# ndjinga/CirculantPreconditioner

Hardware: AMD Instinct MI355X
Metric: PCApply/s on 256^3 complex grid (higher is better)
Workload: dtype c128 (f64 complex); 1 GPU; 256x256x256 c128 circulant PCApply, transport symbol lambda=(0.6, 0.15, 0.02); global_batch=1, parallelism=single GPU

## Files before the change

circulantpreconditioner_amd/csrc/cfp_three_pass.hip:

```cpp
#include "cfp_fft_device.h"
#include "cfp_lane.h"
#include "cfp_three_pass.h"

#include <hip/hip_ext.h>

#ifndef CFP_REAL_MID_XCD
#define CFP_REAL_MID_XCD 1
#endif

#define TP_LAUNCH(K, G, B, S, ...)                                                                    \
  do {                                                                                                \
    if (g_stamp.start || g_stamp.stop)                                                                \
      hipExtLaunchKernelGGL(K, G, B, 0, S, g_stamp.start, g_stamp.stop, 0, __VA_ARGS__);              \
    else                                                                                              \
      hipLaunchKernelGGL(K, G, B, 0, S, __VA_ARGS__);                                                 \
  } while (0)

namespace cfp {

namespace {

__device__ __forceinline__ cd dft4_dif(cd v, int q) {
  const cd p = dpp_c<DPP_XOR2>(v);
  cd t = (q & 2) ? csub(p, v) : cadd(v, p);
  if (q == 3) t = mul_mi(t);
  const cd r = dpp_c<DPP_XOR1>(t);
  return (q & 1) ? csub(r, t) : cadd(t, r);
}
__device__ __forceinline__ cd dft4_dit(cd v, int q) {
  const cd r = dpp_c<DPP_XOR1>(v);
  cd u = (q & 1) ? csub(r, v) : cadd(v, r);
  if (q == 3) u = mul_mi(u);
  const cd p = dpp_c<DPP_XOR2>(u);
  return (q & 2) ? csub(p, u) : cadd(u, p);
}
template <int N2>
__device__ __forceinline__ int brev(int j) {
  if constexpr (N2 == 16) return ((j & 1) << 3) | ((j & 2) << 1) | ((j & 4) >> 1) | (j >> 3);
  return N2 == 4 ? ((j & 1) << 1) | (j >> 1) : ((j & 1) << 2) | (j & 2) | (j >> 2);
}
__device__ __forceinline__ int xcd_unit(int it, int G) {
  const int b = it % G;
  return it - b + (b & 7) * (G >> 3) + (b >> 3);
}

__device__ __forceinline__ int idx(int i) {
  asm volatile("" : "+v"(i));
  return i;
}

template <int FLAGS>
__device__ __forceinline__ unsigned char gload_u8(const unsigned char* p) {
  if constexpr ((FLAGS & F_NT_LD) != 0) return __builtin_nontemporal_load(p);
  return *p;
}

constexpr int r0_of(int n, int pts) { return n > pts ? r0_of(n / pts, pts) : n; }

}

#ifndef CFP_POST_NT
#define CFP_POST_NT 1
#endif
constexpr int kPostLoadFlags = CFP_POST_NT ? F_NT_LD : 0;

enum { PR_NO_Y2 = 1, PR_NO_ZMATH = 2, PR_NO_XCHG = 4, PR_NO_LOAD = 8, PR_NO_STORE = 16,
       PR_PRIO = 32 ,
       PR_ZMAJOR = 64  };

template <bool INV, int FLAGS, int N1, int TN, int PTS = 16, bool XS = true, bool LP = false, int BLK = 0,
          bool XCD = false, int PROBE = 0, int FUSE = 0>
__global__ void __launch_bounds__(N1 * (TN / PTS)) __attribute__((amdgpu_waves_per_eu(4)))
k_tp_rows(const cd* in, cd* out, TPArgs a, int nunits) {
#ifndef CFP_KEXP
  static_assert(PROBE == 0, "timing probes are built in tools/kexp only");
#endif
  constexpr int N2 = TN / N1, TR = TN / PTS, NT = N1 * TR, TY = N1 / PTS;
  constexpr bool PRE = !INV && FUSE == 1, POST = INV && FUSE > 0;
  constexpr int NP = POST ? FUSE : 1;
  static_assert(!POST || NP <= TP_POST_MAX, "post dots: at most TP_POST_MAX vectors");
  static_assert(FUSE == 0 || (BLK == 0 && PROBE == 0), "fused work: natural layout, product kernels");
  constexpr bool BL = BLK > 0;
  constexpr int BX = BL ? BLK : 1, BW = N2 * BX;
  static_assert(!LP || (TY == 2 && TN % 32 == 0), "lane pairs: two threads per column, 32 columns per wave");
  static_assert(!BL || (TR % BX == 0 && ((N2 == 8 && (BX == 4 || BX == 8)) || (N2 == 16 && (BX == 2 || BX == 8)))),
                "blocked layout: 4 or 8 x times 8 y2, or 2 or 8 x times 16 y2");
  constexpr int RS = TN + TN / 16;
  constexpr int F = FLAGS | (XS ? F_SPLIT_LDS : 0) | F_LDS_SYNC;
  constexpr int FA = F & ~F_WAVE_LDS;
  static_assert(!(FLAGS & F_WAVE_LDS) || 64 % TR == 0, "wave-local rows: whole rows per wave");
  __shared__ __attribute__((aligned(16))) double lds[N1 * RS * (XS ? 1 : 2)];
  __shared__ cd tw_l[N1];
  __shared__ cd pre_tab_l[PRE ? 3 * TP_PRE_MAX_CLS : 1];
  __shared__ unsigned pre_mk_l[PRE ? TP_PRE_MAX_CLS + 1 : 1];
  __shared__ const unsigned char* pre_cls_l[1];
  __shared__ cd pre_edge_l[PRE ? NT : 1];
  __shared__ double post_l[POST ? 2 * NP * (NT / 64) : 1];
  __shared__ const cd* post_ptr_l[POST ? NP : 1];
  __shared__ int post_n_l[2];
  const int tid = threadIdx.x;
  if constexpr (POST) {
    for (int i = tid; i < 2 * NP * (NT / 64); i += NT) post_l[i] = 0.0;
    if (tid < NP) post_ptr_l[tid] = a.post_v[tid];
    if (tid == 0) {
      post_n_l[0] = a.post_nv;
      post_n_l[1] = a.post_self;
    }
  }
  for (int i = tid; i < N1; i += NT) tw_l[i] = a.tw[N2 * i];
  if constexpr (PRE) {
    for (int c = tid; c < a.pre_ncls; c += NT) {
      const unsigned mk = a.pre_mask[c];
      unsigned dense = 0;
      pre_tab_l[3 * c] = pre_tab_l[3 * c + 1] = pre_tab_l[3 * c + 2] = make_cd(0.0, 0.0);
      for (int k = 0; k < a.pre_nd; ++k)
        if ((mk >> k) & 1u) {
          const int slot = a.pre_off[k] + 1;
          pre_tab_l[3 * c + slot] = a.pre_tab[c * a.pre_nd + k];
          dense |= 1u << slot;
        }
      pre_mk_l[c] = dense;
    }
    if (tid == 0) {
      unsigned all = 0;
      for (int k = 0; k < a.pre_nd; ++k) all |= 1u << (a.pre_off[k] + 1);
      pre_mk_l[TP_PRE_MAX_CLS] = all | (a.pre_cls_x ? 8u : 0u);
      pre_cls_l[0] = a.pre_cls_x ? a.pre_cls_x : a.pre_cls;
    }
  }
  if constexpr (LP || PRE || POST) __syncthreads();
  const int x0 = LP ? (tid & 31) + 32 * (tid >> 6) : tid % TN, ty0 = LP ? (tid >> 5) & 1 : tid / TN;
  const int r0 = tid / TR, tx0 = tid % TR;
  const int lnyl = a.lnyl ? a.lnyl : ilog2(TN);
  const int nyl = 1 << lnyl;
  const auto crow = [&](int z, int y) -> i64 {
    return (i64)(y >> lnyl) * a.chunk + ((i64)z << lnyl) * TN + (i64)(y & (nyl - 1)) * TN;
  };
  const auto load = [&](int u, cd* v) {
    const int x = idx(x0), ty = idx(ty0);
    if constexpr ((PROBE & PR_NO_LOAD) != 0) {
#pragma unroll
      for (int m = 0; m < PTS; ++m) v[m] = make_cd(x + m, ty + u);
      return;
    }
    if (INV) {
      const cd* const src = BL ? in + crow(u / N2, N2 * ty) + (u % N2) * BX + (x / BX) * BW + x % BX
                               : in + crow(u / N2, u % N2 + N2 * ty) + x;
#pragma unroll
      for (int m = 0; m < PTS; ++m) v[m] = gload<FLAGS>(src + crow(0, N2 * TY * m));
    } else if constexpr (PRE) {
      static_assert(LP, "the fused stencil relies on the lane-pair layout");
      const i64 p0 = (i64)(u / N2) * TN * TN + (i64)TN * (u % N2 + N2 * ty);
      const i64 i0 = p0 + x;
      const int l32 = (int)(threadIdx.x & 31), wv = (int)(threadIdx.x >> 6);
      const unsigned slots = ((volatile unsigned*)pre_mk_l)[TP_PRE_MAX_CLS];
      const bool hm = (slots & 1u) != 0, hp = (slots & 4u) != 0;
      const unsigned char* const cls = ((const unsigned char* const volatile*)pre_cls_l)[0];
      const bool by_x = (slots & 8u) != 0;
      int cl[PTS];
      const int clx = by_x ? (int)gload_u8<FLAGS>(cls + x) : 0;
#pragma unroll
      for (int m = 0; m < PTS; ++m) {
        const i64 i = i0 + (i64)TN * N2 * TY * m;
        v[m] = gload<FLAGS>(in + i);
        cl[m] = by_x ? clx : (int)gload_u8<FLAGS>(cls + i);
      }
      cd edge = make_cd(0.0, 0.0);
      {
        const bool left = l32 < 16;
        int xe = left ? x - l32 - 1 : x - l32 + 32;
        xe = xe < 0 ? 0 : (xe > TN - 1 ? TN - 1 : xe);
        if ((left && hm) || (!left && hp)) edge = gload<FLAGS>(in + p0 + (i64)TN * N2 * TY * (l32 & 15) + xe);
      }
      __builtin_amdgcn_sched_barrier(0);
      cd* const el = pre_edge_l + 64 * wv;
      el[threadIdx.x & 63] = edge;
      __builtin_amdgcn_s_waitcnt(0xc07f);
      __builtin_amdgcn_wave_barrier();
      const auto coefs = [&](int c, cd* t) {
        t[0] = pre_tab_l[3 * c];
        t[1] = pre_tab_l[3 * c + 1];
        t[2] = pre_tab_l[3 * c + 2];
      };
      cd tx[3];
      if (by_x) coefs(clx, tx);
#pragma unroll
      for (int m = 0; m < PTS; ++m) {
        cd t[3];
        if (by_x) {
          t[0] = tx[0], t[1] = tx[1], t[2] = tx[2];
        } else {
          coefs(cl[m], t);
        }
        double ax = 0.0, ay = 0.0;
        const auto acc = [&](cd q, cd b) {
          ax = fma(q.x, b.x, fma(-q.y, b.y, ax));
          ay = fma(q.x, b.y, fma(q.y, b.x, ay));
        };
        if (hm) {
          cd bm = dpp_c<DPP_WAVE_SHR1>(v[m]);
          if (l32 == 0) bm = el[32 * ty + m];
          acc(t[0], bm);
        }
        acc(t[1], v[m]);
        if (hp) {
          cd bp = dpp_c<DPP_WAVE_SHL1>(v[m]);
          if (l32 == 31) bp = el[32 * ty + 16 + m];
          acc(t[2], bp);
        }
        v[m] = make_cd(ax, ay);
      }
    } else {
      const cd* const src = in + (i64)(u / N2) * TN * TN + x + (i64)TN * (u % N2 + N2 * ty);
#pragma unroll
      for (int m = 0; m < PTS; ++m) v[m] = gload<FLAGS>(src + (i64)TN * N2 * TY * m);
    }
    __builtin_amdgcn_sched_barrier(0);
  };
  for (int it = blockIdx.x; it < nunits; it += gridDim.x) {
    int u = XCD ? xcd_unit(it, gridDim.x) : it;
    if constexpr ((PROBE & PR_ZMAJOR) != 0) u = (u % (nunits / N2)) * N2 + u / (nunits / N2);
    cd v[PTS];
    load(u, v);
    if (INV) {
#pragma unroll
      for (int m = 0; m < PTS; ++m) v[m] = cconj(v[m]);
    }
    const auto k1_of = [](int m, int ty) {
      return LP ? (m & (PTS / 2 - 1)) + (PTS / 2) * ty + PTS * (m / (PTS / 2)) : ty + TY * m;
    };
    if constexpr ((PROBE & PR_NO_ZMATH) != 0) {
    } else if constexpr (LP) {
      dft_reg<PTS>(v);
      {
        const int ty = idx(ty0);
#pragma unroll
        for (int k = 1; k < PTS; ++k) v[k] = cmul(v[k], tw_l[k * ty]);
      }
#pragma unroll
      for (int k = 0; k < PTS / 2; ++k) swap_c<5>(v[k], v[k + PTS / 2]);
#pragma unroll
      for (int k = 0; k < PTS / 2; ++k) {
        const cd p = v[k], q = v[k + PTS / 2];
        v[k] = cadd(p, q);
        v[k + PTS / 2] = csub(p, q);
      }
    } else {
      const int x = idx(x0), ty = idx(ty0);
      fft_stages<N1, PTS, r0_of(N1, PTS), false, TN, FA>(v, lds, tw_l, x, ty, true);
      lds_barrier();
    }
    if constexpr (!(PROBE & PR_NO_XCHG)) {
      const int x = idx(x0), ty = idx(ty0), r = idx(r0), tx = idx(tx0);
      if constexpr (XS) {
#pragma unroll
        for (int half = 0; half < 2; ++half) {
#pragma unroll
          for (int m = 0; m < PTS; ++m) lds[k1_of(m, ty) * RS + x + (x >> 4)] = half ? v[m].y : v[m].x;
          lds_barrier();
#pragma unroll
          for (int m = 0; m < PTS; ++m) {
            const int xx = tx + TR * m;
            const double val = lds[r * RS + xx + (xx >> 4)];
            if (half) v[m].y = val; else v[m].x = val;
          }
          lds_barrier();
        }
      } else {
        cd* const lc = reinterpret_cast<cd*>(lds);
#pragma unroll
        for (int m = 0; m < PTS; ++m) lc[k1_of(m, ty) * RS + x + (x >> 4)] = v[m];
        lds_barrier();
#pragma unroll
        for (int m = 0; m < PTS; ++m) {
          const int xx = tx + TR * m;
          v[m] = lc[r * RS + xx + (xx >> 4)];
        }
        lds_barrier();
      }
    }
    {
      const int r = idx(r0), tx = idx(tx0);
      if constexpr (!(PROBE & PR_NO_ZMATH))
        fft_stages<TN, PTS, r0_of(TN, PTS), true, N1, F | F_TW_GLOBAL>(v, lds, a.tw, r, tx, true);
    }
    {
      const int r = idx(r0), tx = idx(tx0);
      const double sc = a.scale, sy = INV ? -sc : sc;
      if constexpr ((PROBE & PR_NO_STORE) != 0) {
        double acc = 0.0;
#pragma unroll
        for (int m = 0; m < PTS; ++m) acc += v[m].x * sc + v[m].y * sy;
        if (acc == 1.2345e300) out[tx] = make_cd(acc, 0.0);
      } else if (BL && !INV) {
        cd* dst = out + crow(u / N2, N2 * r) + (u % N2) * BX + (tx / BX) * BW + tx % BX;
#pragma unroll
        for (int m = 0; m < PTS; ++m) gstore<FLAGS>(dst + TR * N2 * m, make_cd(v[m].x * sc, v[m].y * sy));
      } else {
        const i64 e0 = (INV ? (i64)(u / N2) * TN * TN + (i64)TN * (u % N2 + N2 * r) : crow(u / N2, u % N2 + N2 * r)) + tx;
        cd* dst = out + e0;
#pragma unroll
        for (int m = 0; m < PTS; ++m) {
          v[m] = make_cd(v[m].x * sc, v[m].y * sy);
          gstore<FLAGS>(dst + TR * m, v[m]);
        }
        if constexpr (POST) {
          const int lane = tid & 63, wv = tid >> 6;
          const int pnv = ((volatile int*)post_n_l)[0], pself = ((volatile int*)post_n_l)[1];
          constexpr int QB = 4;
#pragma unroll
          for (int j = 0; j < NP; ++j) {
            if (j < pnv) {
              double sr = 0.0, si = 0.0;
              if ((pself >> j) & 1) {
#pragma unroll
                for (int m = 0; m < PTS; ++m) sr += v[m].x * v[m].x + v[m].y * v[m].y;
              } else {
                const cd* pv = ((const cd* volatile*)post_ptr_l)[j] + e0;
#pragma unroll
                for (int m0 = 0; m0 < PTS; m0 += QB) {
                  cd q[QB];
#pragma unroll
                  for (int m = 0; m < QB; ++m) q[m] = gload<kPostLoadFlags>(pv + TR * (m0 + m));
#pragma unroll
                  for (int m = 0; m < QB; ++m) {
                    const cd w = v[m0 + m];
                    sr += q[m].x * w.x + q[m].y * w.y;
                    si += q[m].x * w.y - q[m].y * w.x;
                  }
                }
              }
              sr = wave_sum_d(sr);
              si = wave_sum_d(si);
              if (lane == 0) {
                post_l[(2 * j) * (NT / 64) + wv] += sr;
                post_l[(2 * j + 1) * (NT / 64) + wv] += si;
              }
            }
          }
        }
      }
    }
    lds_barrier();
  }
  if constexpr (POST) {
    __syncthreads();
    if (tid < 2 * NP) {
      double s = 0.0;
#pragma unroll
      for (int q = 0; q < NT / 64; ++q) s += post_l[tid * (NT / 64) + q];
      a.post_partial[(size_t)blockIdx.x * 16 + tid] = s;
    }
  }
}


template <int FLAGS, int T, int N2, int TN, int PTS = 16, bool XS = true, int NX = TN, bool XCD = false,
          int BLK = 0, int PROBE = 0>
__global__ void __launch_bounds__(T * (TN / PTS)) __attribute__((amdgpu_waves_per_eu(4)))
k_tp_mid(cd* data, TPArgs a, int nunits) {
#ifndef CFP_KEXP
  static_assert(PROBE == 0, "timing probes are built in tools/kexp only");
#endif
  constexpr int N1 = TN / N2, TZ = TN / PTS, NT = T * TZ, XT = T / N2, NXT = NX / XT;
  constexpr int F = FLAGS | (XS ? F_SPLIT_LDS : 0) | F_LDS_SYNC;
  static_assert(N2 == 4 || N2 == 8 || N2 == 16, "the y2 DFT runs across 4, 8 or 16 lanes");
  static_assert(BLK == 0 || (BLK % XT == 0 && NX % BLK == 0), "blocks of whole x tiles");
  __shared__ __attribute__((aligned(16))) double lds[T * TN * (XS ? 1 : 2)];
  __shared__ cd tw_l[TN];
  const int tid = threadIdx.x;
  for (int i = tid; i < TN; i += NT) tw_l[i] = a.tw[i];
  const int c0 = tid & (T - 1), tz0 = tid / T;
  const i64 zs = (i64)NX << (a.lnyl ? a.lnyl : ilog2(TN));
  struct Col {
    cd* col;
    int y2, xk;
    cd w, w8, w16;
  };
  const auto column = [&](int u) {
    int c = c0, tz = tz0;
    asm volatile("" : "+v"(c), "+v"(tz));
    Col q;
    const int xt = u % NXT, k1 = u / NXT;
    q.y2 = c & (N2 - 1);
    q.xk = xt * XT + c / N2;
    q.col = BLK ? data + (i64)NX * N2 * k1 + (q.xk / BLK) * (N2 * BLK) + q.y2 * BLK + q.xk % BLK + zs * tz
                : data + q.xk + (i64)NX * (q.y2 + N2 * k1) + zs * tz;
    q.w = a.tw[(q.y2 * (a.k1_off + k1)) & (TN - 1)];
    q.w8 = a.tw[(TN / 8) * (q.y2 & 3)];
    if constexpr (N2 == 16) q.w16 = a.tw[(TN / 16) * (q.y2 & 7)];
    return q;
  };
  for (int it = blockIdx.x; it < nunits; it += gridDim.x) {
    const int u = XCD ? xcd_unit(it, gridDim.x) : it;
    cd v[PTS];
    {
      const Col q = column(u);
#pragma unroll
      for (int m = 0; m < PTS; ++m) {
        if constexpr (PROBE & PR_NO_LOAD) v[m] = make_cd(c0 + m, tz0 + u);
        else v[m] = gload<FLAGS>(q.col + zs * TZ * m);
      }
#pragma unroll
      for (int m = 0; m < PTS; ++m) {
        v[m] = cmul(v[m], q.w);
        if constexpr ((PROBE & PR_NO_Y2) != 0) continue;
        if constexpr (N2 == 16) {
          const cd p = lane_xor8(v[m]);
          v[m] = (q.y2 & 8) ? cmul(csub(p, v[m]), q.w16) : cadd(v[m], p);
        }
        if constexpr (N2 >= 8) {
          const cd p = lane_xor4(v[m]);
          v[m] = (q.y2 & 4) ? cmul(csub(p, v[m]), q.w8) : cadd(v[m], p);
        }
      }
#pragma unroll
      for (int m = 0; m < PTS; ++m)
        if constexpr (!(PROBE & PR_NO_Y2)) v[m] = dft4_dif(v[m], q.y2 & 3);
    }
    {
      int c = c0, tz = tz0;
      asm volatile("" : "+v"(c), "+v"(tz));
      if constexpr (!(PROBE & PR_NO_ZMATH))
        fft_stages<TN, PTS, r0_of(TN, PTS), false, T, F>(v, lds, tw_l, c, tz, true);
    }
    {
      int c = c0, tz = tz0;
      asm volatile("" : "+v"(c), "+v"(tz));
      const int k1 = a.k1_off + u / NXT, y2 = c & (N2 - 1);
      const cd cs = a.colsym[(u % NXT) * XT + c / N2 + (i64)NX * (k1 + N1 * brev<N2>(y2))];
#pragma unroll
      for (int m = 0; m < PTS; ++m) {
        const cd d = cadd(cadd(cs, a.axsym[tz + TZ * m]), make_cd(1.0, 0.0));
        v[m] = (PROBE & PR_NO_ZMATH) ? cconj(v[m]) : cconj(cdiv_sym(v[m], d));
      }
      if constexpr (!(PROBE & PR_NO_ZMATH)) fft_stages<TN, PTS, r0_of(TN, PTS), false, T, F>(v, lds, tw_l, c, tz, false);
    }
    {
      const Col q = column(u);
#pragma unroll
      for (int m = 0; m < PTS; ++m)
        if constexpr (!(PROBE & PR_NO_Y2)) v[m] = dft4_dit(v[m], q.y2 & 3);
#pragma unroll
      for (int m = 0; m < PTS; ++m) {
        if constexpr ((PROBE & PR_NO_Y2) != 0) {
          v[m] = cmul(v[m], q.w);
          continue;
        }
        if constexpr (N2 >= 8) {
          const cd u = (q.y2 & 4) ? cmul(v[m], q.w8) : v[m];
          const cd p = lane_xor4(u);
          v[m] = (q.y2 & 4) ? csub(p, u) : cadd(u, p);
        }
        if constexpr (N2 == 16) {
          const cd u = (q.y2 & 8) ? cmul(v[m], q.w16) : v[m];
          const cd p = lane_xor8(u);
          v[m] = (q.y2 & 8) ? csub(p, u) : cadd(u, p);
        }
        v[m] = cmul(v[m], q.w);
      }
      if constexpr (PROBE & PR_NO_STORE) {
        double acc = 0.0;
#pragma unroll
        for (int m = 0; m < PTS; ++m) acc += v[m].x + v[m].y;
        if (acc == 1.2345e300) q.col[0] = make_cd(acc, 0.0);
      } else {
#pragma unroll
        for (int m = 0; m < PTS; ++m) gstore<FLAGS>(q.col + zs * TZ * m, cconj(v[m]));
      }
    }
    lds_barrier();
  }
}

namespace {
__device__ __forceinline__ double ror8_d(double v) {
  const long long b = __double_as_longlong(v);
  const int lo = __builtin_amdgcn_mov_dpp((int)(b & 0xffffffffll), 0x128, 0xf, 0xf, false);
  const int hi = __builtin_amdgcn_mov_dpp((int)(b >> 32), 0x128, 0xf, 0xf, false);
  return __longlong_as_double(((long long)hi << 32) | (unsigned int)lo);
}
__device__ __forceinline__ cd bfly_l3(cd v, double sgn) {
  return make_cd(fma(sgn, v.x, ror8_d(v.x)), fma(sgn, v.y, ror8_d(v.y)));
}
}

template <int B, int D, bool TW = true, int NR = 16>
__device__ __forceinline__ void dif_pairs(cd* v, cd w) {
#pragma unroll
  for (int k = 0; k < NR; ++k)
    if ((k & D) == 0) swap_c<B>(v[k], v[k + D]);
#pragma unroll
  for (int k = 0; k < NR; ++k)
    if ((k & D) == 0) {
      const cd a = v[k], b = v[k + D];
      v[k] = cadd(a, b);
      v[k + D] = TW ? cmul(csub(a, b), w) : csub(a, b);
    }
}

typedef __attribute__((address_space(3))) void lds_void_t;
typedef __attribute__((address_space(1))) void glb_void_t;
template <int T, int N2, int TN, int PROBE = 0, bool PF = false, int NX = TN, int ST = 0, int LD = 0, bool BL = false,
          bool XCD = false, int TAG = 0>
__global__ void __launch_bounds__(T * (TN / 16)) __attribute__((amdgpu_waves_per_eu(4)))
k_tp_mid_sw(cd* data, TPArgs a, int nunits) {
#ifndef CFP_KEXP
  static_assert(PROBE == 0, "timing probes are built in tools/kexp only");
#endif
  static_assert(T == 64 || (T == 32 && N2 == 8), "a wave = the 64 columns of one z group, or 32 columns of two");
  static_assert(N2 == 4 || N2 == 8, "y2 = the top 2 or 3 lane bits");
  static_assert(TN == 256, "z = 16 x 16: radix-16 stage A in registers, one exchange, radix-16 stage B");
  constexpr int N1 = TN / N2, TZ = TN / 16, NT = T * TZ, XT = T / N2, NXT = NX / XT;
  constexpr int XB = ilog2(XT);
  static_assert(NX % XT == 0, "whole x tiles");
  static_assert(!BL || (NX == TN && N2 == 8), "blocked layout: complex grid, 8 x times 8 y2");
  __shared__ __attribute__((aligned(16))) double lds[T * TN];
  __shared__ cd tw_l[TN];
  const int tid = threadIdx.x;
  for (int i = tid; i < TN; i += NT) tw_l[i] = a.tw[i];
  __syncthreads();
  const int lane0 = tid & 63;
  const int c0 = T == 64 ? lane0 : (lane0 & 3) | ((lane0 >> 3) << 2);
  const int tz0 = T == 64 ? tid / 64 : 2 * (tid >> 6) + ((lane0 >> 2) & 1);
  const i64 zs = (i64)NX << (a.lnyl ? a.lnyl : ilog2(TN));
  const auto col_ptr = [&](int u, int c, int tz) {
    const int xt = u % NXT, k1 = u / NXT;
    if constexpr (BL) return data + (i64)NX * N2 * k1 + xt * T + c + zs * tz;
    return data + xt * XT + (c & (XT - 1)) + (i64)NX * ((c >> XB) + N2 * k1) + zs * tz;
  };
  const auto tw_y = [&](int u, int c) { return tw_l[((c >> XB) * (a.k1_off + u / NXT)) & (TN - 1)]; };
  constexpr int NPF = PF ? 8 : 0;
  const int wv = __builtin_amdgcn_readfirstlane(tid / 64);
  if constexpr ((PROBE & PR_PRIO) != 0) {
    if (wv >= NT / 128) __builtin_amdgcn_s_setprio(1);
  }
  const auto prefetch = [&](int u) {
    const int c = idx(c0), tz = idx(tz0);
    const cd* src = col_ptr(u, c, tz);
#pragma unroll
    for (int m = 0; m < NPF; ++m)
      __builtin_amdgcn_global_load_lds((glb_void_t*)(src + zs * TZ * m), (lds_void_t*)(lds + (wv * NPF + m) * 128),
                                       16, 0, (LD & F_NT_LD) ? 2 : 0);
  };
  static_assert(!PF || (NT / 64) * NPF * 128 <= T * TN, "the prefetch fits the exchange buffer");
  if constexpr (PF) {
    if ((int)blockIdx.x < nunits) prefetch(XCD ? xcd_unit(blockIdx.x, gridDim.x) : (int)blockIdx.x);
  }
  const auto exchange_t = [&](cd* v, bool first) {
    if constexpr (PROBE & PR_NO_XCHG) return;
    const int c = idx(c0), tz = idx(tz0), lane = idx(lane0);
    const int l3 = N2 == 8 ? ((lane >> 3) & 1) : 0, l4 = (lane >> 4) & 1, l5 = (lane >> 5) & 1;
    const int wbase = (tz * 16 + l5 + 2 * l4) * T + (c & (XT - 1)) + XT * l3;
#pragma unroll
    for (int h = 0; h < 2; ++h) {
      if (!(first && h == 0)) lds_barrier();
#pragma unroll
      for (int r = 0; r < 16; ++r) {
        const int p = N2 == 8 ? 4 * (r & 1) + 2 * ((r >> 1) & 1) : 2 * (r & 1) + ((r >> 1) & 1);
        const int off = (r & 12) * T + XT * (N2 == 8 ? p & 6 : p);
        lds[wbase + off] = h ? v[r].y : v[r].x;
      }
      lds_barrier();
#pragma unroll
      for (int t = 0; t < 16; ++t) {
        const double d = lds[(tz + TZ * t) * T + c];
        if (h) v[t].y = d; else v[t].x = d;
      }
    }
  };
  const auto stage_b = [&](cd* v) {
    if constexpr (PROBE & PR_NO_ZMATH) return;
    const int tz = idx(tz0);
#pragma unroll
    for (int t = 1; t < 16; ++t) v[t] = cmul(v[t], tw_l[tz * t]);
    dft_reg<16>(v);
  };
  const auto lane_sign = [&]() {
    const int lane = idx(lane0);
    return (lane & 8) ? -1.0 : 1.0;
  };

  for (int it = blockIdx.x; it < nunits; it += gridDim.x) {
    const int u = XCD ? xcd_unit(it, gridDim.x) : it;
    cd v[16];
    if constexpr (PROBE & PR_NO_LOAD) {
      const int c = idx(c0), tz = idx(tz0);
#pragma unroll
      for (int m = 0; m < 16; ++m) v[m] = make_cd(c + m, tz + u);
    } else {
      const int c = idx(c0), tz = idx(tz0);
      const cd* src = col_ptr(u, c, tz);
#pragma unroll
      for (int m = NPF; m < 16; ++m) v[m] = gload<LD>(src + zs * TZ * m);
      if constexpr (PF) {
        asm volatile("s_waitcnt vmcnt(0)" ::: "memory");
#pragma unroll
        for (int m = 0; m < NPF; ++m) {
          const int lane = idx(lane0);
          v[m] = fromv(*reinterpret_cast<const dv2*>(lds + (wv * NPF + m) * 128 + 2 * lane));
        }
      }
    }
    {
      const int c = idx(c0);
      const cd w = tw_y(u, c);
#pragma unroll
      for (int m = 0; m < 16; ++m) v[m] = cmul(v[m], w);
    }
    if constexpr (!(PROBE & PR_NO_ZMATH)) dft_reg<16>(v);
    if constexpr (PROBE & PR_NO_Y2) {
    } else if constexpr (N2 == 8) {
      {
        const int lane = idx(lane0);
        dif_pairs<5, 1>(v, tw_l[(TN / 8) * ((lane >> 3) & 3)]);
      }
      {
        const int lane = idx(lane0);
        dif_pairs<4, 2>(v, tw_l[(TN / 4) * ((lane >> 3) & 1)]);
      }
      const double s = lane_sign();
#pragma unroll
      for (int r = 0; r < 16; ++r) v[r] = bfly_l3(v[r], s);
    } else {
      {
        const int lane = idx(lane0);
        dif_pairs<5, 1>(v, tw_l[(TN / 4) * ((lane >> 4) & 1)]);
      }
      dif_pairs<4, 2, false>(v, make_cd(1.0, 0.0));
    }
    exchange_t(v, !PF);
    stage_b(v);
    {
      const int c = idx(c0), tz = idx(tz0);
      const int k1 = a.k1_off + u / NXT, p = c >> XB;
      const cd cs = a.colsym[(u % NXT) * XT + (c & (XT - 1)) + (i64)NX * (k1 + N1 * brev<N2>(p))];
#pragma unroll
      for (int m = 0; m < 16; ++m) {
        const cd d = cadd(cadd(cs, a.axsym[tz + TZ * m]), make_cd(1.0, 0.0));
        v[m] = (PROBE & PR_NO_ZMATH) ? cconj(v[m]) : cconj(cdiv_sym(v[m], d));
      }
    }
    if constexpr (!(PROBE & PR_NO_ZMATH)) dft_reg<16>(v);
    if constexpr (PROBE & PR_NO_Y2) {
    } else if constexpr (N2 == 8) {
      {
        const double s = lane_sign();
#pragma unroll
        for (int r = 0; r < 16; ++r) v[r] = bfly_l3(v[r], s);
      }
      {
        const int lane = idx(lane0);
        const cd w = tw_l[(TN / 4) * ((lane >> 3) & 1)];
#pragma unroll
        for (int k = 0; k < 16; ++k)
// ... 597 lines not shown
        for (int m = 0; m < PTS; ++m) lds[(ty + TY * m) * RS + x + (x >> 4)] = h ? -v[m].y : v[m].x;
        lds_barrier();
#pragma unroll
        for (int t = 0; t < PTS; ++t) {
          const int k = tpc + TPC * t, km = (M - k) & (M - 1);
          const double d = lds[r * RS + k + (k >> 4)], dm = lds[r * RS + km + (km >> 4)];
          if (h) { v[t].y = d; xm[t].y = dm; } else { v[t].x = d; xm[t].x = dm; }
        }
      }
    }
    lds_barrier();
    if (tpc == 0) xm[0] = qy[r];
#pragma unroll
    for (int t = 0; t < PTS; ++t) {
      const int k = tpc + TPC * t;
      const cd e = make_cd(0.5 * (v[t].x + xm[t].x), 0.5 * (v[t].y - xm[t].y));
      const cd d = make_cd(0.5 * (v[t].x - xm[t].x), 0.5 * (v[t].y + xm[t].y));
      const cd o = cmul(d, cconj(a.tw[k]));
      v[t] = cconj(make_cd(e.x - o.y, e.y + o.x));
    }
  };
  for (int u = blockIdx.x; u < nunits; u += gridDim.x) {
    const int z = u / N2, y2 = u % N2;
    cd v[PTS];
    if constexpr (!INV) {
      {
        const int r = idx(r0), tpc = idx(tpc0);
        const cd* src = reinterpret_cast<const cd*>(in_r) + ((i64)z * NY + y2 + N2 * r) * M + tpc;
#pragma unroll
        for (int t = 0; t < PTS; ++t) v[t] = gload<MF>(src + TPC * t);
        __builtin_amdgcn_sched_barrier(0);
        fft_stages<M, PTS, r0_of(M, PTS), true, N1, FW>(v, lds, tw_m, r, tpc, true);
      }
      to_columns_r2c(v, z, y2);
      {
        const int x = idx(x0), ty = idx(ty0);
        fft_stages<N1, PTS, r0_of(N1, PTS), false, TC, FW>(v, lds, tw_1, x, ty, true);
        cd* dst = H + ((i64)z * NY + y2 + N2 * ty) * M + x;
#pragma unroll
        for (int m = 0; m < PTS; ++m) dst[(i64)N2 * TY * M * m] = v[m];
      }
      if constexpr (WL) asm volatile("s_waitcnt lgkmcnt(0)" ::: "memory");
      if (tid < N1) {
        const int k = idx(tid);
        cd acc = make_cd(0.0, 0.0);
#pragma unroll 8
        for (int j = 0; j < N1; ++j) acc = cadd(acc, cmul(qy[j], tw_1[(j * k) & (N1 - 1)]));
        Q[(i64)z * NY + y2 + N2 * k] = acc;
      }
    } else {
      cd qk = make_cd(0.0, 0.0);
      if (tid < N1) qk = Q[(i64)z * NY + y2 + N2 * idx(tid)];
      {
        const int x = idx(x0), ty = idx(ty0);
        const cd* src = H + ((i64)z * NY + y2 + N2 * ty) * M + x;
#pragma unroll
        for (int m = 0; m < PTS; ++m) v[m] = src[(i64)N2 * TY * M * m];
        __builtin_amdgcn_sched_barrier(0);
#pragma unroll
        for (int m = 0; m < PTS; ++m) v[m] = cconj(v[m]);
        fft_stages<N1, PTS, r0_of(N1, PTS), false, TC, FW>(v, lds, tw_1, x, ty, true);
      }
      if (tid < 64) {
        if (tid < N1) qy[tid] = qk;
        asm volatile("s_waitcnt lgkmcnt(0)" ::: "memory");
        cd acc = make_cd(0.0, 0.0);
        const int y1 = idx(tid) & (N1 - 1);
#pragma unroll 8
        for (int k = 0; k < N1; ++k) acc = cadd(acc, cmul(qy[k], cconj(tw_1[(y1 * k) & (N1 - 1)])));
        asm volatile("s_waitcnt lgkmcnt(0)" ::: "memory");
        if (tid < N1) qy[tid] = acc;
      }
      to_rows_c2r(v, z, y2);
      {
        const int r = idx(r0), tpc = idx(tpc0);
        fft_stages<M, PTS, r0_of(M, PTS), true, N1, FW>(v, lds, tw_m, r, tpc, true);
        const double sc = a.scale;
        cd* dst = reinterpret_cast<cd*>(out_r) + ((i64)z * NY + y2 + N2 * r) * M + tpc;
#pragma unroll
        for (int t = 0; t < PTS; ++t) gstore<MF>(dst + TPC * t, make_cd(v[t].x * sc, -v[t].y * sc));
      }
    }
    lds_barrier();
  }
}

hipError_t launch_three_pass_real(int stage, int n, const double* b, cd* H, cd* Q, double* x, const TPArgs& a,
                                  hipStream_t s, bool alt_rows) {
  if (stage == 3) {
    if (n == 128)
      hipLaunchKernelGGL((k_tp_mid<0, 4, 4, 128, 8, false, 1>), dim3(32), dim3(4 * 16), 0, s, Q, a, 32);
    else
      hipLaunchKernelGGL((k_tp_mid<0, 8, 8, 256, 4, false, 1>), dim3(32), dim3(8 * 64), 0, s, Q, a, 32);
    return hipGetLastError();
  }
  if (n == 128) {
    if (stage == 1) {
      constexpr int units = (64 / 8) * 32;
      hipLaunchKernelGGL((k_tp_mid<0, 32, 4, 128, 8, false, 64>), dim3(grid_of(units, 2)), dim3(512), 0, s, H, a,
                         units);
    } else {
      constexpr int units = 128 * 4;
      const unsigned g = grid_of(units, 4);
      if (stage == 0 && alt_rows)
        hipLaunchKernelGGL((k_tp_rows_r2c<false, 64, 32, 4, 128>), dim3(g), dim3(256), 0, s, b, H, Q, nullptr, a,
                           units);
      else if (stage == 0)
        hipLaunchKernelGGL((k_tp_rows_r2c<false, 64, 32, 4, 128, 0, 4, false, true>), dim3(g), dim3(256), 0, s, b, H,
                           Q, nullptr, a, units);
      else if (alt_rows)
        hipLaunchKernelGGL((k_tp_rows_r2c<true, 64, 32, 4, 128>), dim3(g), dim3(256), 0, s, nullptr, H, Q, x, a,
                           units);
      else
        hipLaunchKernelGGL((k_tp_rows_r2c<true, 64, 32, 4, 128, 0, 4, false, true>), dim3(g), dim3(256), 0, s, nullptr,
                           H, Q, x, a, units);
    }
    return hipGetLastError();
  }
  if (stage == 1) {
    constexpr int units = (128 / 8) * 32;
    const unsigned gx = CFP_REAL_MID_XCD ? grid_xcd(units, 1) : 0;
    if (gx)
      hipLaunchKernelGGL((k_tp_mid_sw<64, 8, 256, 0, true, 128, 0, 0, false, true>), dim3(gx), dim3(1024), 0, s, H, a,
                         units);
    else
      hipLaunchKernelGGL((k_tp_mid_sw<64, 8, 256, 0, true, 128>), dim3(grid_of(units, 1)), dim3(1024), 0, s, H, a,
                         units);
  } else {
    constexpr int units = 256 * 8;
    const unsigned g = grid_of(units, 2);
    if (stage == 0 && !alt_rows)
      hipLaunchKernelGGL((k_tp_rows_r2c<false, 128, 32, 8, 256, F_NT_LD, 6, false, true>), dim3(grid_of(units, 3)),
                         dim3(512), 0, s, b, H, Q, nullptr, a, units);
    else if (stage == 0)
      hipLaunchKernelGGL((k_tp_rows_r2c<false, 128, 32, 8, 256, F_NT_LD, 6>), dim3(grid_of(units, 3)), dim3(512), 0, s, b,
                         H, Q, nullptr, a, units);
    else if (!alt_rows)
      hipLaunchKernelGGL((k_tp_rows_r2c<true, 128, 32, 8, 256, F_NT_ST, 4, true, true>), dim3(g), dim3(512), 0, s,
                         nullptr, H, Q, x, a, units);
    else
      hipLaunchKernelGGL((k_tp_rows_r2c<true, 128, 32, 8, 256, F_NT_ST, 4, true>), dim3(g), dim3(512), 0, s, nullptr, H, Q, x, a,
                         units);
  }
  return hipGetLastError();
}


constexpr int kP1Flags = F_NT_LD, kP1InPlaceFlags = 0;
constexpr int kP3Flags = F_NT_ST;
constexpr bool kRowsLP = true;
constexpr int kP2LoadFlags = F_NT_LD;
constexpr bool kRowsWave = true;
constexpr bool kRowsXCD = CFP_ROWS_XCD != 0;

template <int N1, int TN, int PER_CU, int PTS = 16, bool XS = true, bool LP = false, int BL = 0, bool XCD = false,
          int P1F = kP1Flags, int P3F = kP3Flags, bool WR = kRowsWave>
static void launch_rows(int stage, const cd* in, cd* out, const TPArgs& a, hipStream_t s) {
  constexpr int units = TN * (TN / N1);
  constexpr int W = WR ? F_WAVE_LDS : 0;
  const unsigned g = XCD ? grid_xcd(units, PER_CU) : grid_of(units, PER_CU);
  if constexpr (XCD) {
    if (g == 0) {
      launch_rows<N1, TN, PER_CU, PTS, XS, LP, BL, false, P1F, P3F, WR>(stage, in, out, a, s);
      return;
    }
  }
  const dim3 blk(N1 * (TN / PTS));
  if (stage == 0 && in == out)
    TP_LAUNCH((k_tp_rows<false, kP1InPlaceFlags | W, N1, TN, PTS, XS, LP, BL, XCD>), dim3(g), blk, s, in, out, a, units);
  else if (stage == 0)
    TP_LAUNCH((k_tp_rows<false, P1F | W, N1, TN, PTS, XS, LP, BL, XCD>), dim3(g), blk, s, in, out, a, units);
  else
    TP_LAUNCH((k_tp_rows<true, P3F | W, N1, TN, PTS, XS, LP, BL, XCD>), dim3(g), blk, s, in, out, a, units);
}
template <int N1, int TN, int PER_CU, int PTS, bool XS, bool LP, int P1F = kP1Flags, int P3F = kP3Flags,
          bool XCD = kRowsXCD>
static void launch_rows_ab(bool alt, int stage, const cd* in, cd* out, const TPArgs& a, hipStream_t s) {
  if (alt) launch_rows<N1, TN, PER_CU, PTS, XS, LP, 0, XCD, P1F, P3F, !kRowsWave>(stage, in, out, a, s);
  else launch_rows<N1, TN, PER_CU, PTS, XS, LP, 0, XCD, P1F, P3F, kRowsWave>(stage, in, out, a, s);
}

template <int T, int N2, int TN, int PER_CU, int PTS = 16, bool XS = true>
static void launch_mid(cd* data, const TPArgs& a, hipStream_t s) {
  constexpr int units = (TN / (T / N2)) * (TN / N2);
  TP_LAUNCH((k_tp_mid<0, T, N2, TN, PTS, XS>), dim3(grid_of(units, PER_CU)), dim3(T * (TN / PTS)), s, data, a, units);
}

template <int N2, int TN, bool PF = false, bool BL = false, int T = 64>
static void launch_mid_sw(cd* data, const TPArgs& a, hipStream_t s) {
  constexpr int units = (TN / (T / N2)) * (TN / N2);
  if constexpr (T == 64 && N2 == 8 && TN == 256 && PF && !BL) {
    if (a.krylov) {
      TP_LAUNCH((k_tp_mid_sw<T, N2, TN, 0, PF, TN, 0, kP2LoadFlags, BL, false, 1>), dim3(grid_of(units, 64 / T)),
                dim3(T * (TN / 16)), s, data, a, units);
      return;
    }
  }
  TP_LAUNCH((k_tp_mid_sw<T, N2, TN, 0, PF, TN, 0, kP2LoadFlags, BL>), dim3(grid_of(units, 64 / T)),
            dim3(T * (TN / 16)), s, data, a, units);
}

template <bool PF>
static void launch_mid_rec(cd* data, const TPArgs& a, hipStream_t s) {
  constexpr int units = (256 / 8) * (256 / 8);
  if (a.krylov)
    TP_LAUNCH((k_tp_mid_rec<0, PF, kP2LoadFlags, 1>), dim3(grid_of(units, 1)), dim3(1024), s, data, a, units);
  else
    TP_LAUNCH((k_tp_mid_rec<0, PF, kP2LoadFlags>), dim3(grid_of(units, 1)), dim3(1024), s, data, a, units);
}

hipError_t launch_three_pass_rec2(cd* data, const TPArgs& a, const cd* tab2, hipStream_t s) {
  constexpr int units = (256 / 8) * (256 / 8);
  const bool pf = ((uintptr_t)data & 15) == 0;
  const dim3 g(grid_of(units, 1)), b(1024);
  if (a.krylov) {
    if (pf) TP_LAUNCH((k_tp_mid_rec2<0, true, kP2LoadFlags, 1>), g, b, s, data, a, units, tab2);
    else TP_LAUNCH((k_tp_mid_rec2<0, false, kP2LoadFlags, 1>), g, b, s, data, a, units, tab2);
  } else {
    if (pf) TP_LAUNCH((k_tp_mid_rec2<0, true, kP2LoadFlags>), g, b, s, data, a, units, tab2);
    else TP_LAUNCH((k_tp_mid_rec2<0, false, kP2LoadFlags>), g, b, s, data, a, units, tab2);
  }
  return hipGetLastError();
}

bool three_pass_slab_supported(const i64 n[3], int P) {
  const bool cube = n[0] == n[1] && n[1] == n[2] && (n[0] == 256 || n[0] == 512);
  return cube && P >= 1 && P <= 16 && (32 % P) == 0;
}

int three_pass_slab_n2(i64 n) { return n == 512 ? 16 : 8; }

hipError_t launch_three_pass_slab(int stage, int n, const cd* in, cd* out, const TPArgs& a, int nzl, hipStream_t s) {
  if (n == 512) {
    constexpr int W = kRowsWave ? F_WAVE_LDS : 0;
    if (stage == 1) {
      const int nk1 = (1 << a.lnyl) / 16;
      const int units = 256 * nk1;
      const unsigned g = grid_xcd(units, 1);
      if (g) TP_LAUNCH((k_tp_mid<0, 32, 16, 512, 16, true, 512, true>), dim3(g), dim3(1024), s, out, a, units);
      else TP_LAUNCH((k_tp_mid<0, 32, 16, 512, 16, true, 512, false>), dim3(grid_of(units, 1)), dim3(1024), s, out, a,
                     units);
    } else {
      const int units = nzl * 16;
      const unsigned gx = kRowsXCD && units >= (int)grid_of(1 << 30, 1) ? grid_xcd(units, 1) : 0;
      const unsigned g = gx ? gx : grid_of(units, 1);
      if (stage == 0 && gx)
        TP_LAUNCH((k_tp_rows<false, F_NT_LD | W, 32, 512, 16, true, kRowsLP, 0, true>), dim3(g), dim3(1024), s, in, out, a, units);
      else if (stage == 0)
        TP_LAUNCH((k_tp_rows<false, F_NT_LD | W, 32, 512, 16, true, kRowsLP>), dim3(g), dim3(1024), s, in, out, a, units);
      else if (gx)
        TP_LAUNCH((k_tp_rows<true, F_NT_ST | W, 32, 512, 16, true, kRowsLP, 0, true>), dim3(g), dim3(1024), s, in, out, a, units);
      else
        TP_LAUNCH((k_tp_rows<true, F_NT_ST | W, 32, 512, 16, true, kRowsLP>), dim3(g), dim3(1024), s, in, out, a, units);
    }
    return hipGetLastError();
  }
  if (stage == 1) {
    const int nk1 = a.lnyl ? (1 << a.lnyl) / 8 : 32;
    const int units = 32 * nk1;
    if (((uintptr_t)out & 15) == 0)
      hipLaunchKernelGGL((k_tp_mid_sw<64, 8, 256, 0, true, 256, 0, kP2LoadFlags>), dim3(grid_of(units, 1)), dim3(1024), 0, s,
                         out, a, units);
    else
      hipLaunchKernelGGL((k_tp_mid_sw<64, 8, 256, 0, false, 256, 0, kP2LoadFlags>), dim3(grid_of(units, 1)), dim3(1024), 0, s,
                         out, a, units);
  } else {
    const int units = nzl * 8;
    const unsigned gx = kRowsXCD && units >= (int)grid_of(1 << 30, 2) ? grid_xcd(units, 2) : 0;
    const unsigned g = gx ? gx : grid_of(units, 2);
    constexpr int W = kRowsWave ? F_WAVE_LDS : 0;
    if (stage == 0 && gx)
      hipLaunchKernelGGL((k_tp_rows<false, F_NT_LD | W, 32, 256, 16, true, kRowsLP, 0, true>), dim3(g), dim3(512), 0, s,
                         in, out, a, units);
    else if (stage == 0)
      hipLaunchKernelGGL((k_tp_rows<false, F_NT_LD | W, 32, 256, 16, true, kRowsLP>), dim3(g), dim3(512), 0, s,
                         in, out, a, units);
    else if (gx)
      hipLaunchKernelGGL((k_tp_rows<true, F_NT_ST | W, 32, 256, 16, true, kRowsLP, 0, true>), dim3(g), dim3(512), 0, s,
                         in, out, a, units);
    else
      hipLaunchKernelGGL((k_tp_rows<true, F_NT_ST | W, 32, 256, 16, true, kRowsLP>), dim3(g), dim3(512), 0, s,
                         in, out, a, units);
  }
  return hipGetLastError();
}

bool three_pass_fused_supported(int n, TPShape shape) { return n == 256 && shape.n1 == 0 && shape.mid == TP_MID_DEFAULT; }

template <bool XCD>
static void launch_rows_fused(int stage, const cd* in, cd* out, const TPArgs& a, hipStream_t s, unsigned g) {
  constexpr int W = kRowsWave ? F_WAVE_LDS : 0, units = 256 * 8;
  if (stage == 0)
    TP_LAUNCH((k_tp_rows<false, kP1Flags | W, 32, 256, 16, true, kRowsLP, 0, XCD, 0, 1>), dim3(g), dim3(512), s, in,
              out, a, units);
  else
    TP_LAUNCH((k_tp_rows<true, kP3Flags | W, 32, 256, 16, true, kRowsLP, 0, XCD, 0, TP_POST_MAX>), dim3(g), dim3(512),
              s, in, out, a, units);
}

hipError_t launch_three_pass_fused(int stage, int n, const cd* in, cd* out, const TPArgs& a, hipStream_t s,
                                   unsigned* grid_out) {
  if (n != 256 || (stage != 0 && stage != 2)) return hipErrorNotSupported;
  if (stage == 0 && (!a.pre_cls || in == out || a.pre_ncls < 1 || a.pre_ncls > TP_PRE_MAX_CLS || a.pre_nd < 1 ||
                     a.pre_nd > 3))
    return hipErrorInvalidValue;
  if (stage == 2 && (a.post_nv < 1 || a.post_nv > TP_POST_MAX || !a.post_partial)) return hipErrorInvalidValue;
  constexpr int units = 256 * 8;
  const unsigned gx = kRowsXCD ? grid_xcd(units, 2) : 0;
  const unsigned g = gx ? gx : grid_of(units, 2);
  if (grid_out) *grid_out = g;
  if (gx) launch_rows_fused<true>(stage, in, out, a, s, g);
  else launch_rows_fused<false>(stage, in, out, a, s, g);
  return hipGetLastError();
}

bool three_pass_zrec_shape(int n, TPShape shape) {
  return n == 256 && shape.mid == TP_MID_DEFAULT && (shape.n1 == 0 || shape.n1 == 32);
}

bool three_pass_shape_valid(int n1, int mid, i64 n) {
  if (mid == TP_MID_ROWSALT) return n1 == 0;
  if (n1 == 16) return n == 128 && mid >= TP_MID_DEFAULT && mid <= TP_MID_SWAP64;
  return (n1 == 0 || n1 == 32 || n1 == 64) && (mid >= 0 && mid <= TP_MID_SWAP32X) &&
         !(mid >= TP_MID_BLOCKED && n1 == 64);
}

hipError_t launch_three_pass(int stage, int n, const cd* in, cd* out, const TPArgs& a, TPShape shape,
                             hipStream_t s) {
  const bool ra = shape.mid == TP_MID_ROWSALT;
  if (ra) shape.mid = TP_MID_DEFAULT;
  if (n == 100) return launch_three_pass_sq(stage, n, in, out, a, shape, s);
  if (n == 512) {
    const bool bl = shape.mid == TP_MID_BLOCKED, bl8 = shape.mid == TP_MID_BLOCKED32;
    if (stage == 1) {
      constexpr int units = (512 / 2) * 32;
      const unsigned g = grid_xcd(units, 1);
      if (g == 0) return hipErrorNotSupported;
      if (bl) TP_LAUNCH((k_tp_mid<0, 32, 16, 512, 16, true, 512, true, 2>), dim3(g), dim3(1024), s, out, a, units);
      else if (bl8) TP_LAUNCH((k_tp_mid<0, 32, 16, 512, 16, true, 512, true, 8>), dim3(g), dim3(1024), s, out, a, units);
      else TP_LAUNCH((k_tp_mid<0, 32, 16, 512, 16, true, 512, true>), dim3(g), dim3(1024), s, out, a, units);
    } else if (bl) {
      launch_rows<32, 512, 1, 16, true, kRowsLP, 2, true>(stage, in, out, a, s);
    } else if (bl8) {
      launch_rows<32, 512, 1, 16, true, kRowsLP, 8>(stage, in, out, a, s);
    } else if (shape.mid == TP_MID_LANE64) {
      launch_rows<32, 512, 1>(stage, in, out, a, s);
    } else {
      launch_rows_ab<32, 512, 1, 16, true, kRowsLP>(ra, stage, in, out, a, s);
    }
    return hipGetLastError();
  }
  if (n == 128) {
    const int n1 = shape.n1 ? shape.n1 : (shape.mid == TP_MID_LANE64 || shape.mid == TP_MID_SWAP64 ? 32 : 16);
    if (n1 == 16) {
      if (stage == 1) {
        if (shape.mid == TP_MID_LANE32) launch_mid<64, 8, 128, 1, 8, false>(out, a, s);
        else if (shape.mid == TP_MID_LANE64) launch_mid<64, 8, 128, 1>(out, a, s);
        else if (shape.mid == TP_MID_SWAP64) launch_mid<64, 8, 128, 1, 16, false>(out, a, s);
        else {
          constexpr int units = (128 / 4) * 16;
          const unsigned g = grid_xcd(units, 2);
          if (g) TP_LAUNCH((k_tp_mid<0, 32, 8, 128, 8, false, 128, true>), dim3(g), dim3(512), s, out, a, units);
          else launch_mid<32, 8, 128, 2, 8, false>(out, a, s);
        }
      } else {
        launch_rows_ab<16, 128, 4, 8, false, true, 0, 0, false>(ra, stage, in, out, a, s);
      }
      return hipGetLastError();
    }
    if (shape.mid == TP_MID_LANE64) {
      if (stage == 1) launch_mid<64, 4, 128, 2>(out, a, s);
      else launch_rows<32, 128, 4>(stage, in, out, a, s);
    } else {
      if (stage == 1) launch_mid<32, 4, 128, 2, 8, false>(out, a, s);
      else if (shape.mid == TP_MID_SWAP64) launch_rows<32, 128, 2, 8, false>(stage, in, out, a, s);
      else launch_rows<32, 128, 2, 8, false, false, 0, false, 0, 0>(stage, in, out, a, s);
    }
    return hipGetLastError();
  }
  const int n1 = shape.n1 == 64 ? 64 : 32;
  const bool t32 = shape.mid == TP_MID_LANE32;
  const bool pf_ok = ((uintptr_t)out & 15) == 0;
  if (shape.mid == TP_MID_BLOCKED) {
    if (stage != 1) launch_rows<32, 256, 2, 16, true, kRowsLP, 8>(stage, in, out, a, s);
    else if (pf_ok) launch_mid_sw<8, 256, true, true>(out, a, s);
    else launch_mid_sw<8, 256, false, true>(out, a, s);
    return hipGetLastError();
  }
  if (shape.mid == TP_MID_SWAP32X) {
    if (stage != 1) {
      launch_rows<32, 256, 2, 16, true, kRowsLP>(stage, in, out, a, s);
    } else {
      constexpr int units = (256 / 4) * 32;
      const unsigned g = grid_xcd(units, 2);
      if (g == 0) return hipErrorNotSupported;
      if (pf_ok)
        TP_LAUNCH((k_tp_mid_sw<32, 8, 256, 0, true, 256, 0, kP2LoadFlags, false, true>), dim3(g), dim3(512), s, out, a,
                  units);
      else
        TP_LAUNCH((k_tp_mid_sw<32, 8, 256, 0, false, 256, 0, kP2LoadFlags, false, true>), dim3(g), dim3(512), s, out, a,
                  units);
    }
    return hipGetLastError();
  }
  if (shape.mid == TP_MID_BLOCKED32) {
    if (stage != 1) launch_rows<32, 256, 2, 16, true, kRowsLP, 4, true>(stage, in, out, a, s);
    else if (pf_ok) launch_mid_sw<8, 256, true, true, 32>(out, a, s);
    else launch_mid_sw<8, 256, false, true, 32>(out, a, s);
    return hipGetLastError();
  }
  if (stage == 1) {
    if (a.zrec && three_pass_zrec_shape(n, shape)) {
      if (pf_ok) launch_mid_rec<true>(out, a, s);
      else launch_mid_rec<false>(out, a, s);
    } else if ((shape.mid == TP_MID_SWAP64_PF || shape.mid == TP_MID_DEFAULT) && pf_ok) {
      if (n1 == 64) launch_mid_sw<4, 256, true>(out, a, s);
      else launch_mid_sw<8, 256, true>(out, a, s);
    } else if (shape.mid == TP_MID_SWAP64 || shape.mid == TP_MID_SWAP64_PF || shape.mid == TP_MID_DEFAULT) {
      if (n1 == 64) launch_mid_sw<4, 256>(out, a, s);
      else launch_mid_sw<8, 256>(out, a, s);
    } else if (n1 == 64) {
      if (t32) launch_mid<32, 4, 256, 2>(out, a, s);
      else launch_mid<64, 4, 256, 1>(out, a, s);
    } else if (t32) {
      launch_mid<32, 8, 256, 2>(out, a, s);
    } else {
      launch_mid<64, 8, 256, 1>(out, a, s);
    }
  } else if (n1 == 64) {
    launch_rows<64, 256, 1>(stage, in, out, a, s);
  } else {
    launch_rows_ab<32, 256, 2, 16, true, kRowsLP>(ra, stage, in, out, a, s);
  }
  return hipGetLastError();
}

}
```

Before: 3716 PCApply/s.

## Prefetch next rows tile into LDS via global_load_lds in 256^3 row passes

Adds a software-pipelined path for the 256^3 row-FFT passes (first and third stages). Each wave issues asynchronous global-to-LDS loads for the first NPF slots of its next work unit before storing the current unit's results, then reads them from LDS on the next iteration while loading the remaining slots directly. The aim is to hide global load latency behind the current tile's stores and compute. In exchange it reuses part of the wave's LDS rows as a staging buffer, which needs an extra barrier before the exchange and a full vmcnt wait, and it only runs for aligned inputs with the XCD, wave-LDS and lane-pair settings enabled.

```diff
diff --git a/circulantpreconditioner_amd/csrc/cfp_three_pass.hip b/circulantpreconditioner_amd/csrc/cfp_three_pass.hip
--- a/circulantpreconditioner_amd/csrc/cfp_three_pass.hip
+++ b/circulantpreconditioner_amd/csrc/cfp_three_pass.hip
@@ -68,13 +68,54 @@
        PR_PRIO = 32 ,
        PR_ZMAJOR = 64  };
 
+typedef __attribute__((address_space(3))) void lds_void_t;
+typedef __attribute__((address_space(1))) void glb_void_t;
+namespace rows {
+struct Tile {
+  static constexpr int TN = 256, N2 = 8;
+  const cd* in;
+  int wv;
+  double* pf_l;
+  static __device__ __forceinline__ unsigned lane_off(int x, int ty) {
+    return 16u * ((unsigned)(x & 31) + (unsigned)(TN * N2) * (unsigned)ty);
+  }
+  static __device__ __forceinline__ const cd* at(const cd* base, unsigned off) {
+    return reinterpret_cast<const cd*>(reinterpret_cast<const char*>(base) + off);
+  }
+  __device__ __forceinline__ const cd* slot_ptr(int u, int m) const {
+    i64 e = (i64)(u / N2) * TN * TN + (u % N2) * TN + 32 * wv + 2 * TN * N2 * m;
+    asm volatile("" : "+s"(e));
+    return in + e;
+  }
+  template <int NPF, int LD>
+  __device__ __forceinline__ void prefetch(int u, unsigned loff) const {
+    asm volatile("" : "+s"(u), "+v"(loff));
+#pragma unroll
+    for (int m = 0; m < NPF; ++m)
+      __builtin_amdgcn_global_load_lds((glb_void_t*)at(slot_ptr(u, m), loff), (lds_void_t*)(pf_l + m * 128), 16, 0,
+                                       (LD & (F_NT | F_NT_LD)) ? 2 : 0);
+  }
+  __device__ __forceinline__ cd prefetched(int m, int lane) const {
+    return fromv(*reinterpret_cast<const dv2*>(pf_l + m * 128 + 2 * lane));
+  }
+  template <int LD>
+  __device__ __forceinline__ cd load(int u, int m, unsigned loff) const {
+    return gload<LD>(at(slot_ptr(u, m), loff));
+  }
+};
+}
+
 template <bool INV, int FLAGS, int N1, int TN, int PTS = 16, bool XS = true, bool LP = false, int BLK = 0,
-          bool XCD = false, int PROBE = 0, int FUSE = 0>
+          bool XCD = false, int PROBE = 0, int FUSE = 0, int NPF = 0>
 __global__ void __launch_bounds__(N1 * (TN / PTS)) __attribute__((amdgpu_waves_per_eu(4)))
 k_tp_rows(const cd* in, cd* out, TPArgs a, int nunits) {
 #ifndef CFP_KEXP
   static_assert(PROBE == 0, "timing probes are built in tools/kexp only");
 #endif
+  constexpr bool PF = NPF > 0;
+  static_assert(!PF || (N1 == 32 && TN == 256 && PTS == 16 && XS && LP && BLK == 0 && FUSE == 0 &&
+                        (FLAGS & F_WAVE_LDS) != 0 && NPF <= 8),
+                "prefetch: the one-GPU 256^3 sweeps, at most 8 slots in the wave's own rows");
   constexpr int N2 = TN / N1, TR = TN / PTS, NT = N1 * TR, TY = N1 / PTS;
   constexpr bool PRE = !INV && FUSE == 1, POST = INV && FUSE > 0;
   constexpr int NP = POST ? FUSE : 1;
@@ -217,11 +258,40 @@
     }
     __builtin_amdgcn_sched_barrier(0);
   };
+  const auto pf_tile = [&]() {
+    const int wv = __builtin_amdgcn_readfirstlane(idx(x0) >> 5);
+    return rows::Tile{in, wv, lds + wv * (4 * RS)};
+  };
+  static_assert(!PF || (NPF * 128 <= 4 * RS && (4 * RS) % 2 == 0), "the prefetch fits the wave's rows, 16-byte aligned");
+  static_assert(!PF || !(PROBE & PR_ZMAJOR), "prefetch: blockIdx or XCD unit order");
+  if constexpr (PF && !(PROBE & PR_NO_LOAD)) {
+    if ((int)blockIdx.x < nunits)
+      pf_tile().template prefetch<NPF, FLAGS>(XCD ? xcd_unit(blockIdx.x, gridDim.x) : (int)blockIdx.x,
+                                              rows::Tile::lane_off(idx(x0), idx(ty0)));
+  }
   for (int it = blockIdx.x; it < nunits; it += gridDim.x) {
     int u = XCD ? xcd_unit(it, gridDim.x) : it;
     if constexpr ((PROBE & PR_ZMAJOR) != 0) u = (u % (nunits / N2)) * N2 + u / (nunits / N2);
     cd v[PTS];
-    load(u, v);
+    if constexpr (PF && !(PROBE & PR_NO_LOAD)) {
+      const rows::Tile tile = pf_tile();
+      {
+        int ul = u;
+        unsigned lo = rows::Tile::lane_off(idx(x0), idx(ty0));
+        asm volatile("" : "+s"(ul), "+v"(lo));
+#pragma unroll
+        for (int m = NPF; m < PTS; ++m) v[m] = tile.template load<FLAGS>(ul, m, lo);
+      }
+      asm volatile("s_waitcnt vmcnt(0)" ::: "memory");
+      {
+        const int lane = (idx(x0) & 31) + 32 * idx(ty0);
+#pragma unroll
+        for (int m = 0; m < NPF; ++m) v[m] = tile.prefetched(m, lane);
+      }
+      __builtin_amdgcn_sched_barrier(0);
+    } else {
+      load(u, v);
+    }
     if (INV) {
 #pragma unroll
       for (int m = 0; m < PTS; ++m) v[m] = cconj(v[m]);
@@ -250,6 +320,7 @@
       fft_stages<N1, PTS, r0_of(N1, PTS), false, TN, FA>(v, lds, tw_l, x, ty, true);
       lds_barrier();
     }
+    if constexpr (PF) lds_barrier();
     if constexpr (!(PROBE & PR_NO_XCHG)) {
       const int x = idx(x0), ty = idx(ty0), r = idx(r0), tx = idx(tx0);
       if constexpr (XS) {
@@ -292,6 +363,11 @@
 #pragma unroll
         for (int m = 0; m < PTS; ++m) acc += v[m].x * sc + v[m].y * sy;
         if (acc == 1.2345e300) out[tx] = make_cd(acc, 0.0);
+        if constexpr (PF && !(PROBE & PR_NO_LOAD)) {
+          const int nx = it + (int)gridDim.x;
+          if (nx < nunits)
+            pf_tile().template prefetch<NPF, FLAGS>(XCD ? xcd_unit(nx, gridDim.x) : nx, rows::Tile::lane_off(idx(x0), idx(ty0)));
+        }
       } else if (BL && !INV) {
         cd* dst = out + crow(u / N2, N2 * r) + (u % N2) * BX + (tx / BX) * BW + tx % BX;
 #pragma unroll
@@ -299,10 +375,26 @@
       } else {
         const i64 e0 = (INV ? (i64)(u / N2) * TN * TN + (i64)TN * (u % N2 + N2 * r) : crow(u / N2, u % N2 + N2 * r)) + tx;
         cd* dst = out + e0;
-#pragma unroll
-        for (int m = 0; m < PTS; ++m) {
-          v[m] = make_cd(v[m].x * sc, v[m].y * sy);
-          gstore<FLAGS>(dst + TR * m, v[m]);
+        if constexpr (PF) {
+#pragma unroll
+          for (int m = 0; m < PTS; ++m) v[m] = make_cd(v[m].x * sc, v[m].y * sy);
+#pragma unroll
+          for (int m = 0; m < PTS; ++m) asm volatile("" : "+v"(v[m].x), "+v"(v[m].y));
+          __builtin_amdgcn_sched_barrier(0);
+          if constexpr (!(PROBE & PR_NO_LOAD)) {
+            const int nx = it + (int)gridDim.x;
+            if (nx < nunits)
+              pf_tile().template prefetch<NPF, FLAGS>(XCD ? xcd_unit(nx, gridDim.x) : nx, rows::Tile::lane_off(idx(x0), idx(ty0)));
+            __builtin_amdgcn_sched_barrier(0);
+          }
+#pragma unroll
+          for (int m = 0; m < PTS; ++m) gstore<FLAGS>(dst + TR * m, v[m]);
+        } else {
+#pragma unroll
+          for (int m = 0; m < PTS; ++m) {
+            v[m] = make_cd(v[m].x * sc, v[m].y * sy);
+            gstore<FLAGS>(dst + TR * m, v[m]);
+          }
         }
         if constexpr (POST) {
           const int lane = tid & 63, wv = tid >> 6;
@@ -341,7 +433,7 @@
         }
       }
     }
-    lds_barrier();
+    if constexpr (!PF) lds_barrier();
   }
   if constexpr (POST) {
     __syncthreads();
@@ -499,8 +591,6 @@
     }
 }
 
-typedef __attribute__((address_space(3))) void lds_void_t;
-typedef __attribute__((address_space(1))) void glb_void_t;
 template <int T, int N2, int TN, int PROBE = 0, bool PF = false, int NX = TN, int ST = 0, int LD = 0, bool BL = false,
           bool XCD = false, int TAG = 0>
 __global__ void __launch_bounds__(T * (TN / 16)) __attribute__((amdgpu_waves_per_eu(4)))
@@ -1404,6 +1494,11 @@
 constexpr int kP2LoadFlags = F_NT_LD;
 constexpr bool kRowsWave = true;
 constexpr bool kRowsXCD = CFP_ROWS_XCD != 0;
+#ifndef CFP_ROWS_PF
+#define CFP_ROWS_PF 8
+#endif
+constexpr int kRowsNPF = CFP_ROWS_PF;
+static_assert(kRowsNPF == 0 || (kRowsNPF >= 4 && kRowsNPF <= 8), "CFP_ROWS_PF: 0 (off) or 4 to 8 slots");
 
 template <int N1, int TN, int PER_CU, int PTS = 16, bool XS = true, bool LP = false, int BL = 0, bool XCD = false,
           int P1F = kP1Flags, int P3F = kP3Flags, bool WR = kRowsWave>
@@ -1577,6 +1672,26 @@
          !(mid >= TP_MID_BLOCKED && n1 == 64);
 }
 
+static unsigned rows_pf_grid(const cd* in, const TPArgs& a) {
+  if (kRowsNPF == 0 || !kRowsXCD || !kRowsWave || !kRowsLP || a.lnyl != 0) return 0;
+  if (((uintptr_t)in & 15) != 0) return 0;
+  return grid_xcd(256 * 8, 2);
+}
+static void launch_rows_pf(int stage, const cd* in, cd* out, const TPArgs& a, hipStream_t s, unsigned g) {
+  if constexpr (kRowsNPF > 0) {
+    constexpr int W = F_WAVE_LDS, units = 256 * 8;
+    if (stage == 0 && in == out)
+      TP_LAUNCH((k_tp_rows<false, kP1InPlaceFlags | W, 32, 256, 16, true, true, 0, true, 0, 0, kRowsNPF>), dim3(g),
+                dim3(512), s, in, out, a, units);
+    else if (stage == 0)
+      TP_LAUNCH((k_tp_rows<false, kP1Flags | W, 32, 256, 16, true, true, 0, true, 0, 0, kRowsNPF>), dim3(g), dim3(512), s,
+                in, out, a, units);
+    else
+      TP_LAUNCH((k_tp_rows<true, kP3Flags | W, 32, 256, 16, true, true, 0, true, 0, 0, kRowsNPF>), dim3(g), dim3(512), s,
+                in, out, a, units);
+  }
+}
+
 hipError_t launch_three_pass(int stage, int n, const cd* in, cd* out, const TPArgs& a, TPShape shape,
                              hipStream_t s) {
   const bool ra = shape.mid == TP_MID_ROWSALT;
@@ -1681,6 +1796,8 @@
     }
   } else if (n1 == 64) {
     launch_rows<64, 256, 1>(stage, in, out, a, s);
+  } else if (const unsigned gpf = ra ? 0 : rows_pf_grid(in, a)) {
+    launch_rows_pf(stage, in, out, a, s, gpf);
   } else {
     launch_rows_ab<32, 256, 2, 16, true, kRowsLP>(ra, stage, in, out, a, s);
   }
```

Result: faster. 3853 PCApply/s (median of 6 runs) (+3.7%).
